# emma-mens/adam-compression

Hardware: AMD Instinct MI355X
Metric: grad elements/s per DGC step (HBM GB/s % of peak), 0.1% ratio, 1-8 GPUs (higher is better)
Workload: dtype f32

## Files before the change

adam-compression_amd/csrc/dgc_common.hpp:

```cpp
#pragma once

#include <hip/hip_runtime.h>
#include <hip/hip_fp16.h>

#include <cstdint>
#include <cstdio>
#include <string>

#include "dgc_hip.h"

namespace dgc {

void set_error(const char* fmt, ...);

#define DGC_FAIL(code, ...)            \
    do {                               \
        ::dgc::set_error(__VA_ARGS__); \
        return (code);                 \
    } while (0)

#define DGC_HIP(call)                                                                  \
    do {                                                                               \
        hipError_t _e = (call);                                                        \
        if (_e != hipSuccess)                                                          \
// ... 170 lines not shown

__host__ __device__ __forceinline__ float bf16_to_f32(uint16_t b) {
    union { uint32_t u; float f; } c{(uint32_t)b << 16};
    return c.f;
}
__host__ __device__ __forceinline__ uint16_t f32_to_bf16(float x) {
    union { float f; uint32_t u; } c{x};
    if ((c.u & 0x7FFFFFFFu) > 0x7F800000u) return (uint16_t)0x7FC0u;
    return (uint16_t)((c.u + 0x7FFFu + ((c.u >> 16) & 1u)) >> 16);
}
__device__ __forceinline__ float f16_to_f32(uint16_t h) { return (float)__builtin_bit_cast(_Float16, h); }
__device__ __forceinline__ uint16_t f32_to_f16(float x) {
    asm volatile("" : "+v"(x));
    return __builtin_bit_cast(uint16_t, (_Float16)x);
}
template <int DT>
__device__ __forceinline__ float h16_to_f32(uint16_t v) { return DT == DGC_BF16 ? bf16_to_f32(v) : f16_to_f32(v); }
template <int DT>
__device__ __forceinline__ uint16_t f32_to_h16(float x) { return DT == DGC_BF16 ? f32_to_bf16(x) : f32_to_f16(x); }
template <int DT>
__device__ __forceinline__ float round16(float x) { return h16_to_f32<DT>(f32_to_h16<DT>(x)); }
__device__ __forceinline__ float thr_mul(float t, float f, int td) {
    const float p = __fmul_rn(t, f);
    return td == DGC_BF16 ? round16<DGC_BF16>(p) : td == DGC_F16 ? round16<DGC_F16>(p) : p;
}

__device__ __forceinline__ void store_value(void* out, int64_t pos, float x, int vdtype) {
    if (vdtype == DGC_BF16)
        reinterpret_cast<uint16_t*>(out)[pos] = f32_to_bf16(x);
    else if (vdtype == DGC_F16)
        reinterpret_cast<__half*>(out)[pos] = __float2half_rn(x);
    else
        reinterpret_cast<float*>(out)[pos] = x;
}

__device__ __forceinline__ void store_index(void* out, int64_t pos, int64_t idx, int idtype) {
    if (idtype == DGC_I32)
        reinterpret_cast<int32_t*>(out)[pos] = (int32_t)idx;
    else
        reinterpret_cast<int64_t*>(out)[pos] = idx;
}

__device__ __forceinline__ uint64_t block_exclusive_scan(uint64_t v, uint64_t* lds16, uint64_t* total) {
    const int lane = threadIdx.x & 63, wid = threadIdx.x >> 6;
    const uint64_t incl = wave_incl_scan64(v);
    if (lane == 63) lds16[wid] = incl;
    __syncthreads();
    uint64_t wbase = 0, tot = 0;
    for (int w = 0; w < (int)(blockDim.x >> 6); ++w) {
        const uint64_t s = lds16[w];
        if (w < wid) wbase += s;
        tot += s;
    }
    __syncthreads();
    *total = tot;
    return wbase + incl - v;
}

}

namespace dgc {
typedef float f4v __attribute__((ext_vector_type(4)));

__device__ __forceinline__ float4 ld_nt(const float4* p) {
    const f4v x = __builtin_nontemporal_load(reinterpret_cast<const f4v*>(p));
    return make_float4(x[0], x[1], x[2], x[3]);
}

__device__ __forceinline__ void st_nt(float4* p, const float4& v) {
    const f4v x = {v.x, v.y, v.z, v.w};
    __builtin_nontemporal_store(x, reinterpret_cast<f4v*>(p));
}

constexpr int64_t kWriteThroughMax = 48LL << 20;
inline bool write_through(int64_t elements) { return elements <= kWriteThroughMax; }

__device__ __forceinline__ void st_stream(float4* p, const float4& v, bool wt) {
    if (wt) {
        const f4v x = {v.x, v.y, v.z, v.w};
        asm volatile("global_store_dwordx4 %0, %1, off sc1\n\ts_nop 1" : : "v"(p), "v"(x) : "memory");
    } else {
        st_nt(p, v);
    }
}
}

namespace dgc {
struct SampleSpec {
    float* out;
    int64_t start;
    int64_t stride;
    int64_t count;
    double inv_stride;
    float inv_stride_f;
};

__device__ __forceinline__ void divmod_u32(uint32_t t, uint32_t s, float inv, uint32_t& q, uint32_t& r) {
    if (s < (1u << 23)) {
        q = (uint32_t)__fmul_rn((float)t, inv);
        int32_t rr = (int32_t)(t - q * s);
        if (rr < 0) {
            q -= 1;
            rr += (int32_t)s;
        } else if (rr >= (int32_t)s) {
            q += 1;
            rr -= (int32_t)s;
        }
        r = (uint32_t)rr;
    } else {
        q = t / s;
        r = t - q * s;
    }
}

__device__ __forceinline__ void floor_divmod_fast(int64_t d, int64_t s, double inv, int64_t& q, int64_t& r) {
    q = (int64_t)floor((double)d * inv);
    r = d - q * s;
    while (r < 0) {
        r += s;
        q -= 1;
    }
    while (r >= s) {
        r -= s;
        q += 1;
    }
}

template <bool NEST, bool ACC>
__device__ __forceinline__ float comp1(float g, float& m, float& v, float mom) {
    if (NEST) {
        m = __fmul_rn(__fadd_rn(m, g), mom);
        if (ACC) {
            v = __fadd_rn(__fadd_rn(v, m), g);
            return v;
        }
        return __fadd_rn(m, g);
    }
    m = __fadd_rn(__fmul_rn(m, mom), g);
    if (ACC) {
        v = __fadd_rn(v, m);
        return v;
    }
    return m;
}

struct ClipArg {
    const float* tab;
    float value;
};

__host__ __device__ inline bool clip_kind_ok(int kind) { return kind >= DGC_CLIP_NONE && kind <= DGC_CLIP_CLAMP; }

template <int CLIP>
__device__ __forceinline__ float clip_coef(const ClipArg& ca, int t) {
    if (CLIP == DGC_CLIP_NONE) return 0.f;
    return ca.tab ? ca.tab[t] : ca.value;
}

template <int CLIP>
__device__ __forceinline__ float clip1(float g, float c) {
    if (CLIP == DGC_CLIP_SCALE) return c < 1.f ? __fmul_rn(g, c) : g;
    if (CLIP == DGC_CLIP_CLAMP) return c != c ? c : (g != g ? g : fminf(fmaxf(g, -c), c));
    return g;
}

template <int CLIP>
// ... 93 lines not shown
```

adam-compression_amd/csrc/select.hip:

```cpp
#include <algorithm>
#include <cstdlib>
#include <cstring>
#include <cmath>
#include <vector>

#include "select_types.hpp"
#include "select_layout.hpp"
#include "select_tiles.hpp"
#include "select_k1.hpp"
#include "select_state.hpp"
#include "select_thresholds.hpp"
#include "select_count.hpp"
#include "select_emit.hpp"
#include "select_heap.hpp"
#include "select_set.hpp"
#include "select_nth.hpp"

namespace dgc {

int64_t payload_layout(int64_t capacity, int vd, int id, int64_t* voff, int64_t* ioff);

__global__ void k_spec_reset(float* spec, int32_t T) {
    for (int i = threadIdx.x; i < kSpecWords * T; i += blockDim.x) spec[i] = __builtin_huge_valf();
}
// ... 316 lines not shown
    OneTable ot{};
    one_layout(*p, 1, 1, false, L, ot);
    SelWS w;
    DGC_TRY(carve_checked(ws, ws_bytes, L, "dgc_select", w));
    w.spec = nullptr;
    w.thr = const_cast<float*>(thr0);
    hipLaunchKernelGGL(k_put_one, dim3(1), dim3(64), 0, s, w, ot);
    DGC_LAUNCHED();
    return select_core(vec, mmt, cfg_of(*p), L, values, indices, count_out, info, w, 0, sync_mode, 1.f,
                       p->status_sink, p->order_out, s);
}

static size_t kth_ws_bytes(int64_t n) { return n <= kSmallN ? 256 : align_up(sizeof(RSState), 256); }

int kth_largest(const float* x, int64_t n, int64_t k, float* out, void* ws, size_t ws_bytes, hipStream_t s) {
    if (!x || !out || n < 1 || k < 1 || k > n)
        DGC_FAIL(DGC_ERR_INVALID, "dgc_kth_largest: need 1 <= k <= n (k=%lld n=%lld)", (long long)k,
                 (long long)n);
    if (n <= kSmallN) {
        hipLaunchKernelGGL(k_rs_small, dim3(1), dim3(kScanThreads), 0, s, x, n, (uint64_t)k, out);
        DGC_LAUNCHED();
        return DGC_OK;
    }
    if (!ws || ws_bytes < sizeof(RSState) || (reinterpret_cast<uintptr_t>(ws) & 255))
        DGC_FAIL(DGC_ERR_WORKSPACE, "dgc_kth_largest: workspace needs %zu bytes", sizeof(RSState));
    RSState* st = reinterpret_cast<RSState*>(ws);
    hipLaunchKernelGGL(k_rs_init, dim3(1), dim3(kBlock), 0, s, st, (uint64_t)k);
    DGC_LAUNCHED();
    return radix_select_passes(DenseKeys{x, n, st, out}, grid_for(n, kBlock * 16, 512), s);
}

static int thresholds(const SelWS& w, const Layout& L, const float* vec, hipStream_t s, int64_t ks1 = 0) {
    if (L.nsmall + L.nwins) {
        hipLaunchKernelGGL(k_rs_small_multi, dim3((unsigned)(L.nsmall + L.nwins)), dim3(kScanThreads), 0, s, w, vec,
                           ks1, L.nsmall);
        DGC_LAUNCHED();
    }
    if (L.grid[BT_SAMP] > 0) {
        if (L.nplain) {
            hipLaunchKernelGGL(k_rs_reset_samples, dim3((unsigned)L.T), dim3(kBlock), 0, s, w, ks1);
            DGC_LAUNCHED();
        }
        const int grid = (int)L.grid[BT_SAMP];
        hipLaunchKernelGGL(k_rs_passes<SampleKeys>, dim3((unsigned)std::min(grid, 1024)), dim3(kBlock), 0, s,
                           SampleKeys{w, vec}, grid, (int)L.T);
        DGC_LAUNCHED();
    }
    return DGC_OK;
}

int compensate(const float* grad, float* mmt, float* vec, float* out, int64_t n, float momentum,
               bool nesterov, bool accumulate, float* samples, int64_t s_start, int64_t s_stride,
               int64_t s_count, hipStream_t st);
int compensate_clip(const float* grad, float* mmt, float* vec, float* out, int64_t n, float momentum,
                    bool nesterov, bool accumulate, float* samples, int64_t s_start, int64_t s_stride,
                    int64_t s_count, int32_t clip_kind, ClipArg ca, hipStream_t st);
int sample_strided_launch(const float* vec, int64_t start, int64_t stride, int64_t count, float* out,
                          hipStream_t s);

static int compress_check(const dgc_select_params* p, void* values, void* indices, int64_t s_start,
                          int64_t s_stride, int64_t top_k_samples, bool need_outputs) {
    if (need_outputs) DGC_TRY(validate_select(p, values, indices));
    else if (!p) DGC_FAIL(DGC_ERR_INVALID, "dgc_compress: null params");
    else if (p->resample) DGC_TRY(check_replay_width(p->numel, p->num_selects, "dgc_compress"));
    const bool sampled = p->numel != p->num_samples;
    if (sampled && (s_stride < 2 || s_start < 0 || s_start >= s_stride))
        DGC_FAIL(DGC_ERR_INVALID, "dgc_compress: sample_start must be in [0, stride)");
    const int64_t cnt = sampled ? ceil_div(p->numel - s_start, s_stride) : p->numel;
    if (need_outputs && (top_k_samples < 1 || top_k_samples > cnt))
        DGC_FAIL(DGC_ERR_INVALID, "dgc_compress: top_k_samples %lld outside [1, %lld]", (long long)top_k_samples,
                 (long long)cnt);
    return DGC_OK;
}

static int one_ws(const dgc_select_params* p, int64_t s_start, int64_t s_stride, int64_t ks, float* spec,
                  void* ws, size_t ws_bytes, Layout& L, SelWS& w, OneTable& ot) {
    one_layout(*p, s_stride, ks, true, L, ot);
    ot.start = p->numel != p->num_samples ? s_start : 0;
    DGC_TRY(carve_checked(ws, ws_bytes, L, "dgc_compress", w));
    w.spec = spec;
    return DGC_OK;
}

template <bool NEST, bool ONE, typename... Args>
static void launch_k1_clip(int32_t clip_kind, dim3 gd, hipStream_t s, Args... args) {
    if (clip_kind == DGC_CLIP_SCALE)
        hipLaunchKernelGGL((k_compensate_list<NEST, ONE, DGC_CLIP_SCALE>), gd, dim3(kBlock), 0, s, args...);
    else if (clip_kind == DGC_CLIP_CLAMP)
        hipLaunchKernelGGL((k_compensate_list<NEST, ONE, DGC_CLIP_CLAMP>), gd, dim3(kBlock), 0, s, args...);
    else
        hipLaunchKernelGGL((k_compensate_list<NEST, ONE, DGC_CLIP_NONE>), gd, dim3(kBlock), 0, s, args...);
}

template <bool ONE, typename... Args>
static void launch_k1(bool nesterov, int32_t clip_kind, dim3 gd, hipStream_t s, Args... args) {
    if (nesterov) launch_k1_clip<true, ONE>(clip_kind, gd, s, args...);
    else launch_k1_clip<false, ONE>(clip_kind, gd, s, args...);
}

static int k1_clip_check(int32_t kind, const float* clip, const char* who) {
    if (!clip_kind_ok(kind)) DGC_FAIL(DGC_ERR_INVALID, "%s: clip kind %d", who, (int)kind);
    if (kind == DGC_CLIP_SCALE && !clip) DGC_FAIL(DGC_ERR_INVALID, "%s: DGC_CLIP_SCALE needs the coefficient table", who);
    return DGC_OK;
}

int compress_begin(const float* grad, float* mmt, float* vec, float momentum, bool nesterov, int64_t s_start,
                   int64_t s_stride, const dgc_select_params* p, float* spec, void* ws, size_t ws_bytes,
                   hipStream_t s, int32_t clip_kind = DGC_CLIP_NONE, ClipArg ca = ClipArg{nullptr, 0.f}) {
    DGC_TRY(compress_check(p, nullptr, nullptr, s_start, s_stride, 1, false));
    DGC_TRY(k1_clip_check(clip_kind, ca.tab, "dgc_compress"));
    if (!grad || !mmt || !vec) DGC_FAIL(DGC_ERR_INVALID, "dgc_compress: null grad/mmt/vec");
    Layout L;
    SelWS w;
    OneTable ot{};
    DGC_TRY(one_ws(p, s_start, s_stride, 1, spec, ws, ws_bytes, L, w, ot));
    const int64_t n = p->numel;
    const bool sampled = n != p->num_samples;
    const int64_t cnt = sampled ? ceil_div(n - s_start, s_stride) : 0;
    const bool list_path = aligned16(grad) && aligned16(mmt) && aligned16(vec) &&
                           (!sampled || (s_stride >= 4 && s_stride < (1LL << 30)));
    if (!list_path) {
        hipLaunchKernelGGL(k_put_one, dim3(1), dim3(64), 0, s, w, ot);
        DGC_LAUNCHED();
        DGC_TRY(mask_flush(vec, mmt, L, w, s));
        DGC_TRY(compensate_clip(grad, mmt, vec, nullptr, n, momentum, nesterov, true, sampled ? w.samples : nullptr,
                                s_start, s_stride, cnt, clip_kind, ca, s));
        hipLaunchKernelGGL(k_no_lists, dim3(1), dim3(64), 0, s, w);
        DGC_LAUNCHED();
        return DGC_OK;
    }
    if (L.grid[BT_K1] > 0x7FFFFFFFLL) DGC_FAIL(DGC_ERR_INVALID, "dgc_compress: n too large");
    if (L.grid[BT_K1] > 0) {
        StartChunk one{};
        one.count = 1;
        one.start[0] = ot.start;
        launch_k1<true>(nesterov, clip_kind, dim3((unsigned)L.grid[BT_K1]), s, grad, mmt, vec, momentum, w, one,
                        (int)write_through(n), ot, ca);
        DGC_LAUNCHED();
    } else {
        hipLaunchKernelGGL(k_put_one, dim3(1), dim3(64), 0, s, w, ot);
        DGC_LAUNCHED();
    }
    if (n & 3) {
        const int64_t done = (n / 4) * 4;
        DGC_TRY(compensate_clip(grad + done, mmt + done, vec + done, nullptr, n - done, momentum, nesterov, true,
                                nullptr, 0, 1, 0, clip_kind, ca, s));
        if (sampled) {
            const int64_t q_first = done >= s_start ? ceil_div(done - s_start, s_stride) : 0;
            const int64_t c = cnt - q_first;
            if (c > 0)
                DGC_TRY(sample_strided_launch(vec, s_start + q_first * s_stride, s_stride, c, w.samples + q_first, s));
        }
    }
    return DGC_OK;
}

int compress_finish(float* vec, float* mmt, int64_t s_start, int64_t s_stride, int64_t top_k_samples,
                    const dgc_select_params* p, float* spec, float margin, void* values, void* indices,
                    int64_t* count_out, dgc_select_info* info, void* ws, size_t ws_bytes, int sync_mode,
                    hipStream_t s) {
    DGC_TRY(compress_check(p, values, indices, s_start, s_stride, top_k_samples, true));
    if (!vec || (p->masking && !mmt)) DGC_FAIL(DGC_ERR_INVALID, "dgc_compress: null vec/mmt");
    Layout L;
    SelWS w;
    OneTable ot{};
    DGC_TRY(one_ws(p, s_start, s_stride, top_k_samples, spec, ws, ws_bytes, L, w, ot));
    DGC_TRY(thresholds(w, L, vec, s, top_k_samples));
    dgc_select_params q = *p;
    q.update_memory = p->update_memory == 2 ? 2 : 1;
    return select_core(vec, mmt, cfg_of(q), L, values, indices, count_out, info, w, 1, sync_mode, margin,
                       p->status_sink, p->order_out, s);
}

static int batch_layout(const dgc_batch_desc* b, HostTables& h) {
    if (!b || b->count < 1 || !b->numel || !b->offset || !b->num_selects || !b->num_samples || !b->top_k_samples ||
        !b->sample_stride)
        DGC_FAIL(DGC_ERR_INVALID, "dgc_batch: null or empty tensor table");
    std::vector<TensorIn> in(b->count);
    int64_t prev_end = 0;
    for (int32_t t = 0; t < b->count; ++t) {
        TensorIn& x = in[t];
        x.n = b->numel[t];
        x.off = b->offset[t];
        x.k = b->num_selects[t];
        x.S = b->num_samples[t];
        x.ks = b->top_k_samples[t];
        x.stride = b->sample_stride[t];
        x.upper_count = (int64_t)std::floor((double)x.k * b->upper_bound);
        x.lower_count = (int64_t)std::ceil(b->lower_bound * (double)x.k);
        x.samples = true;
        if (x.n < 1 || x.k < 1 || x.k > x.n || x.S < 1 || x.S > x.n || x.ks < 1 || x.ks > x.S)
            DGC_FAIL(DGC_ERR_INVALID, "dgc_batch: tensor %d: bad numel/num_selects/num_samples/top_k_samples", t);
        if (b->resample) {
            char who[48];
            std::snprintf(who, sizeof(who), "dgc_batch: tensor %d", t);
            DGC_TRY(check_replay_width(x.n, x.k, who));
        }
        if (x.n != x.S && (x.stride < 4 || x.stride >= (1LL << 30)))
            DGC_FAIL(DGC_ERR_INVALID, "dgc_batch: tensor %d: sample stride %lld outside [4, 2^30)", t,
                     (long long)x.stride);
        if (x.off % kSeg || x.off < prev_end)
            DGC_FAIL(DGC_ERR_INVALID,
                     "dgc_batch: tensor %d: offset %lld must be a multiple of %d, ascending, non-overlapping", t,
                     (long long)x.off, kSeg);
        prev_end = x.off + (int64_t)align_up((size_t)x.n, 4);
        if (prev_end > b->flat_numel) DGC_FAIL(DGC_ERR_INVALID, "dgc_batch: tensor %d past flat_numel", t);
    }
    if (b->int32_indices && b->flat_numel > 2147483647LL)
        DGC_FAIL(DGC_ERR_OVERFLOW, "dgc_batch: int32 indices cannot address %lld elements", (long long)b->flat_numel);
    if (b->dtype != DGC_F32 && b->dtype != DGC_BF16 && b->dtype != DGC_F16)
        DGC_FAIL(DGC_ERR_DTYPE, "dgc_batch: dtype must be DGC_F32, DGC_BF16 or DGC_F16");
    h.build(in.data(), b->count, true);
    return DGC_OK;
}

static SelCfg cfg_of_batch(const dgc_batch_desc* b) {
    const bool half = b->dtype == DGC_BF16 || b->dtype == DGC_F16;
    return SelCfg{(float)b->upper_bound, (float)b->lower_bound, b->max_iters, b->resample, b->momentum_masking,
                  b->fp16_values ? DGC_F16 : (half ? b->dtype : DGC_F32), b->int32_indices ? DGC_I32 : DGC_I64,
                  half ? 0 : (b->deferred_masking ? 2 : 1), half ? b->dtype : DGC_F32,
// ... 15 lines not shown
}

int batch_init(const dgc_batch_desc* b, void* ws, size_t ws_bytes, hipStream_t s) {
    HostTables h;
    SelWS w;
    DGC_TRY(batch_ws(b, ws, ws_bytes, "dgc_batch_init", h, w));
    const Layout& L = h.L;
    DGC_HIP(hipMemsetAsync(w.st, 0, sizeof(SelState) * L.T, s));
    DGC_HIP(hipMemsetAsync(w.setg, 0, sizeof(SetG) * L.T, s));
    DGC_HIP(hipMemsetAsync(w.chain, 0, kChainWords * sizeof(uint32_t), s));
    DGC_HIP(hipMemsetAsync(w.samples, 0, sizeof(float) * L.nsamp, s));
    DGC_HIP(hipMemcpyAsync(w.td, h.td.data(), sizeof(TDesc) * L.T, hipMemcpyHostToDevice, s));
    for (int which = 0; which < BT_COUNT; ++which)
        DGC_HIP(hipMemcpyAsync(w.bt[which], h.bt[which].data(), sizeof(int32_t) * (L.T + 1), hipMemcpyHostToDevice, s));
    if (L.nsmall + L.nwins)
        DGC_HIP(hipMemcpyAsync(w.small, h.small.data(), sizeof(int32_t) * (L.nsmall + L.nwins),
                               hipMemcpyHostToDevice, s));
    hipLaunchKernelGGL(k_spec_reset, dim3(1), dim3(256), 0, s, w.spec, L.T);
    DGC_LAUNCHED();
    DGC_HIP(hipStreamSynchronize(s));
    return DGC_OK;
}

static int check_starts(const HostTables& h, const int64_t* starts, const char* who) {
    for (int32_t t = 0; t < h.L.T; ++t)
        if (h.td[t].samp_off >= 0 && (starts[t] < 0 || starts[t] >= h.td[t].stride))
            DGC_FAIL(DGC_ERR_INVALID, "%s: tensor %d: sample start outside [0, stride)", who, t);
    return DGC_OK;
}

static StartChunk start_chunk(const HostTables& h, const int64_t* starts, const float* const* grads, int32_t first) {
    StartChunk c{};
    c.first = first;
    c.count = std::min<int32_t>(64, h.L.T - first);
    c.ptrs = grads ? 1 : 0;
    for (int i = 0; i < c.count; ++i) {
        c.start[i] = h.td[first + i].samp_off >= 0 ? starts[first + i] : 0;
        c.grad[i] = grads ? grads[first + i] : nullptr;
    }
    return c;
}

static int put_starts(const HostTables& h, const int64_t* starts, const float* const* grads, const SelWS& w,
                      hipStream_t s) {
    for (int32_t t0 = 0; t0 < h.L.T; t0 += 64) {
        hipLaunchKernelGGL(k_put_starts, dim3(1), dim3(64), 0, s, w, start_chunk(h, starts, grads, t0));
        DGC_LAUNCHED();
    }
    return DGC_OK;
}

static int batch_select_core(const dgc_batch_desc* b, const SelCfg& cfg, const HostTables& h, float* vec, float* mmt,
                             void* payload, dgc_select_info* info, const SelWS& w, int sync_mode, hipStream_t s) {
    int64_t cap = 0;
    for (const TDesc& d : h.td) cap += d.k;
    int64_t voff = 0, ioff = 0;
    payload_layout(cap, cfg.vdtype, cfg.idtype, &voff, &ioff);
    char* pl = static_cast<char*>(payload);
    return select_core(vec, mmt, cfg, h.L, pl + voff, pl + ioff, reinterpret_cast<int64_t*>(pl), info, w, 1,
                       sync_mode, b->spec_margin, b->status_sink, reinterpret_cast<int64_t*>(pl) + 1, s);
}

int batch_compress_begin(const dgc_batch_desc* b, const float* grad, const float* const* grads, float* mmt,
                         float* vec, const int64_t* starts, void* ws, size_t ws_bytes, hipStream_t s,
                         int32_t clip_kind = DGC_CLIP_NONE, ClipArg ca = ClipArg{nullptr, 0.f}) {
    HostTables h;
    SelWS w;
    DGC_TRY(k1_clip_check(clip_kind, ca.tab, "dgc_batch_compress"));
    DGC_TRY(batch_ws(b, ws, ws_bytes, "dgc_batch_compress", h, w));
    const Layout& L = h.L;
    if ((!grad && !grads) || !mmt || !vec || !starts) DGC_FAIL(DGC_ERR_INVALID, "dgc_batch_compress: null pointer");
    if ((grad && !aligned16(grad)) || !aligned16(mmt) || !aligned16(vec))
        DGC_FAIL(DGC_ERR_INVALID, "dgc_batch_compress: flat buffers must be 16-B aligned");
    if (grads)
        for (int32_t t = 0; t < L.T; ++t)
            if (!grads[t] || !aligned16(grads[t]))
                DGC_FAIL(DGC_ERR_INVALID, "dgc_batch_compress: gradient %d is null or not 16-B aligned", t);
    DGC_TRY(check_starts(h, starts, "dgc_batch_compress"));
    StartChunk arg{};
    arg.ptrs = grads ? 1 : 0;
    if (L.T <= 64) arg = start_chunk(h, starts, grads, 0);
    else DGC_TRY(put_starts(h, starts, grads, w, s));
    if (L.grid[BT_K1] > 0x7FFFFFFFLL) DGC_FAIL(DGC_ERR_INVALID, "dgc_batch_compress: too many segments");
    launch_k1<false>(b->nesterov != 0, clip_kind, dim3((unsigned)L.grid[BT_K1]), s, grad, mmt, vec, b->momentum, w, arg,
                     (int)write_through(L.nseg * kSeg), OneTable{}, ca);
    DGC_LAUNCHED();
    return DGC_OK;
}

int batch_compress_finish(const dgc_batch_desc* b, float* mmt, float* vec, void* payload, dgc_select_info* info,
                          void* ws, size_t ws_bytes, int sync_mode, hipStream_t s) {
    HostTables h;
    SelWS w;
    DGC_TRY(batch_ws(b, ws, ws_bytes, "dgc_batch_compress", h, w));
    if (!mmt || !vec || !payload) DGC_FAIL(DGC_ERR_INVALID, "dgc_batch_compress: null pointer");
    DGC_TRY(thresholds(w, h.L, vec, s));
    return batch_select_core(b, cfg_of_batch(b), h, vec, mmt, payload, info, w, sync_mode, s);
}

__global__ void __launch_bounds__(kBlock) k_batch_sample(SelWS w, const float* __restrict__ x_flat) {
    const int t = blockIdx.y;
    const TDesc d = w.td[t];
    if (d.samp_off < 0) return;
    const int64_t start = w.starts[t], cnt = w.scnt[t];
    const float* x = x_flat + d.off + start;
    float* out = w.samples + d.samp_off;
    for (int64_t q = (int64_t)blockIdx.x * kBlock + threadIdx.x; q < cnt; q += (int64_t)gridDim.x * kBlock)
        out[q] = fabsf(x[q * d.stride]);
}

int batch_select(const dgc_batch_desc* b, float* vec32, float* mmt32, const int64_t* starts, void* payload,
                 dgc_select_info* info, void* ws, size_t ws_bytes, int sync_mode, hipStream_t s) {
    HostTables h;
    SelWS w;
    DGC_TRY(batch_ws(b, ws, ws_bytes, "dgc_batch_select", h, w));
    const Layout& L = h.L;
    if (!vec32 || !starts || !payload) DGC_FAIL(DGC_ERR_INVALID, "dgc_batch_select: null pointer");
    const SelCfg cfg = cfg_of_batch(b);
    if (cfg.update_memory && cfg.masking && !mmt32) DGC_FAIL(DGC_ERR_INVALID, "dgc_batch_select: masking needs mmt");
    DGC_TRY(check_starts(h, starts, "dgc_batch_select"));
    DGC_TRY(put_starts(h, starts, nullptr, w, s));
    int64_t smax = 0;
    for (const TDesc& d : h.td) smax = std::max(smax, d.samp_off >= 0 ? d.S + 1 : 0);
    if (smax > 0) {
        hipLaunchKernelGGL(k_batch_sample, dim3((unsigned)std::min<int64_t>(ceil_div(smax, (int64_t)kBlock), 1024),
                                                (unsigned)L.T), dim3(kBlock), 0, s, w, vec32);
        DGC_LAUNCHED();
    }
    hipLaunchKernelGGL(k_no_lists, dim3(1), dim3(256), 0, s, w);
    DGC_LAUNCHED();
    DGC_TRY(thresholds(w, L, vec32, s));
    return batch_select_core(b, cfg, h, vec32, mmt32, payload, info, w, sync_mode, s);
}

int batch_compress(const dgc_batch_desc* b, const float* grad, float* mmt, float* vec, const int64_t* starts,
                   void* payload, dgc_select_info* info, void* ws, size_t ws_bytes, int sync_mode, hipStream_t s) {
    if (!payload) DGC_FAIL(DGC_ERR_INVALID, "dgc_batch_compress: null pointer");
    DGC_TRY(batch_compress_begin(b, grad, nullptr, mmt, vec, starts, ws, ws_bytes, s));
    return batch_compress_finish(b, mmt, vec, payload, info, ws, ws_bytes, sync_mode, s);
}

int compress_flush(float* vec, float* mmt, int64_t s_stride, const dgc_select_params* p, void* ws, size_t ws_bytes,
                   hipStream_t s) {
    if (!p || !vec) DGC_FAIL(DGC_ERR_INVALID, "dgc_compress_flush: null params/vec");
    Layout L;
    SelWS w;
    OneTable ot{};
    DGC_TRY(one_ws(p, 0, s_stride, 1, nullptr, ws, ws_bytes, L, w, ot));
    return mask_flush(vec, mmt, L, w, s);
}

int batch_flush(const dgc_batch_desc* b, float* mmt, float* vec, void* ws, size_t ws_bytes, hipStream_t s) {
    HostTables h;
    SelWS w;
    DGC_TRY(batch_ws(b, ws, ws_bytes, "dgc_batch_flush", h, w, vec && mmt));
    return mask_flush(vec, mmt, h.L, w, s);
}

}

extern "C" size_t dgc_kth_largest_workspace(int64_t n) { return dgc::kth_ws_bytes(n); }

extern "C" int dgc_kth_largest(const float* x, int64_t n, int64_t k, float* thr_out, void* ws,
                               size_t ws_bytes, void* stream) {
    return dgc::kth_largest(x, n, k, thr_out, ws, ws_bytes, static_cast<hipStream_t>(stream));
}

// ... 154 lines not shown
```

adam-compression_amd/csrc/select_k1.hpp:

```cpp
#pragma once
#include "select_tiles.hpp"

namespace dgc {
template <bool NEST, bool ONE, int CLIP>
__global__ void __launch_bounds__(kBlock)
k_compensate_list(const float* __restrict__ g_flat, float* __restrict__ mmt_flat, float* __restrict__ vec_flat,
                  float mom, SelWS w, StartChunk sc, int wt, OneTable ot, ClipArg ca) {
    const int t = ONE ? 0 : task(w, BT_K1, blockIdx.x);
    const TDesc d = ONE ? ot.d : w.td[t];
    const int lane = threadIdx.x & 63, wave = threadIdx.x >> 6;
    const int64_t b0 = ONE ? 0 : w.bt[BT_K1][t];
    const int64_t ls = ((int64_t)blockIdx.x - b0) * kSegPerBlock4 + wave;
    if (ONE && blockIdx.x == 0 && threadIdx.x == 0) {
        w.td[0] = ot.d;
        for (int which = 0; which < BT_COUNT; ++which) {
            w.bt[which][0] = ot.bt[which][0];
            w.bt[which][1] = ot.bt[which][1];
        }
        w.small[0] = 0;
    }
    const bool arg_start = t < sc.count;
    const float* gsrc = !sc.ptrs ? g_flat + d.off : (arg_start ? sc.grad[t] : w.gptr[t]);
    const float4* g = reinterpret_cast<const float4*>(gsrc);
    float4* mmt = reinterpret_cast<float4*>(mmt_flat + d.off);
    float4* vec = reinterpret_cast<float4*>(vec_flat + d.off);
    const int64_t n4 = d.nv4, n = d.n;
    const float tl = w.spec ? w.spec[kSpecWords * t] : __builtin_huge_valf();
    SelState* st = w.st + t;
    if (blockIdx.x == b0 && threadIdx.x == 0) st->t_list = tl;
    const bool sample = d.samp_off >= 0;
    const int64_t start = !sample ? 0 : (arg_start ? sc.start[t] : w.starts[t]);
    const int64_t scount = !sample ? 0 : (arg_start ? ceil_div(d.n - start, d.stride) : w.scnt[t]);
    if (arg_start && blockIdx.x == b0 && threadIdx.x == 0) {
        w.starts[t] = sc.start[t];
        w.scnt[t] = sample ? scount : d.n;
    }
    float* sout = sample ? w.samples + d.samp_off : nullptr;
    float* win = w.samples + d.win_off;
    const float tw = w.spec ? w.spec[kSpecWords * t + 2] : __builtin_huge_valf();
    const uint32_t win_key = abs_key(tw < __builtin_huge_valf() ? tw : tl);
    const bool windowed = sample && d.win_cap > 0;
    uint32_t* win_cnt = &st->win_cnt[st->epoch & 1];
    uint32_t* whist = reinterpret_cast<uint32_t*>(w.samples + d.whist_off);
    if (windowed && blockIdx.x == b0 && threadIdx.x == 0) st->win_key = win_key;
    int64_t q0 = 0, r0 = 0;
    if (sample) floor_divmod_fast(ls * kSeg - start, d.stride, d.inv_stride, q0, r0);
    float4 gv[kSegTiles], mv[kSegTiles], vv[kSegTiles];
    const float cf = clip_coef<CLIP>(ca, t);
#pragma unroll
    for (int u = 0; u < kSegTiles; ++u) {
        const int64_t v = ls * (kSeg / 4) + u * 64 + lane;
        if (v < n4) {
            gv[u] = clip4<CLIP>(sc.ptrs && 4 * v + 3 >= n ? ld_tail4(gsrc, 4 * v, n) : ld_nt(g + v), cf);
            mv[u] = ld_nt(mmt + v);
            vv[u] = ld_nt(vec + v);
        }
    }
    uint32_t c = 0, mk = 0;
    const int64_t seg = d.seg0 + ls;
    uint16_t* lo = w.lst_off;
    float* lv = w.lst_val;
    if (st->def_mode && ls < d.nseg) apply_deferred_mask(*st, w, d, ls, lane, vv, mv);
#pragma unroll
    for (int u = 0; u < kSegTiles; ++u) {
        const int64_t v = ls * (kSeg / 4) + u * 64 + lane;
        const bool ok = v < n4;
        float x[4] = {0.f, 0.f, 0.f, 0.f};
        uint32_t valid = 0;
        bool hit = false;
        float hv = 0.f;
        if (ok) {
            x[0] = comp1<NEST, true>(gv[u].x, mv[u].x, vv[u].x, mom);
            x[1] = comp1<NEST, true>(gv[u].y, mv[u].y, vv[u].y, mom);
            x[2] = comp1<NEST, true>(gv[u].z, mv[u].z, vv[u].z, mom);
            x[3] = comp1<NEST, true>(gv[u].w, mv[u].w, vv[u].w, mom);
            st_stream(mmt + v, mv[u], wt);
            st_stream(vec + v, vv[u], wt);
            const int64_t e = 4 * v;
            valid = e + 3 < n ? 0xFu : (e + 2 < n ? 7u : (e + 1 < n ? 3u : (e < n ? 1u : 0u)));
            if (sample) {
                const uint32_t tt = (uint32_t)r0 + 4u * (uint32_t)(u * 64 + lane);
                const uint32_t s32 = (uint32_t)d.stride;
                uint32_t q1, r;
                divmod_u32(tt, s32, d.inv_stride_f, q1, r);
                const uint32_t j = r == 0 ? 0u : s32 - r;
                if (j < 4 && ((valid >> j) & 1u)) {
                    const int64_t qi = q0 + q1 + (r == 0 ? 0 : 1);
                    if (qi >= 0 && qi < scount) {
                        hv = fabsf(x[j]);
                        sout[qi] = hv;
                        hit = windowed && __float_as_uint(hv) >= win_key;
                    }
                }
            }
        }
        const uint64_t hb = __ballot(hit);
        if (hb) {
            const int leader = __ffsll((unsigned long long)hb) - 1;
            uint32_t base = 0;
            if (lane == leader) base = atomicAdd(win_cnt, (uint32_t)__popcll(hb));
            base = __shfl(base, leader);
            const uint32_t pos = base + (uint32_t)__popcll(hb & ((1ull << lane) - 1));
            if (hit && pos < (uint64_t)d.win_cap) win[pos] = hv;
            if (hit) atomicAdd(&whist[win_bin(__float_as_uint(hv), win_key)], 1u);
        }
        list_append(ge_mask(x, valid, tl), x, u * 256, c, lo, lv, seg);
        mk = max(mk, tile_max_key(x, valid));
    }
    const bool spilled = c > (uint32_t)kCap;
    mk = wave_max(mk);
    if (lane == 0 && ls < d.nseg) {
        const bool tail = d.tail && ls == d.nseg - 1;
        w.seg_lcnt[seg] = tail ? lcnt_pack(kCap + 1, 0xFFFFu) : lcnt_pack(c, lmax_code(mk));
    }
    const uint64_t any = __ballot(spilled);
    __shared__ uint32_t nsp;
    if (threadIdx.x == 0) nsp = 0;
    __syncthreads();
    if (lane == 0 && any) atomicAdd(&nsp, 1u);
    __syncthreads();
    if (threadIdx.x == 0 && nsp) atomicAdd(&st->spill[st->epoch & 1][blockIdx.x % kSpillShards], nsp);
}

__global__ void k_no_lists(SelWS w) {
    for (int t = threadIdx.x; t < w.T; t += blockDim.x) w.st[t].t_list = __builtin_huge_valf();
}
}
```

adam-compression_amd/csrc/select_tiles.hpp:

```cpp
#pragma once
#include "select_layout.hpp"

namespace dgc {
__device__ __forceinline__ float4 ld_tail4(const float* __restrict__ g, int64_t e0, int64_t n) {
    if (e0 + 3 < n) return ld_nt(reinterpret_cast<const float4*>(g + e0));
    return make_float4(g[e0], e0 + 1 < n ? g[e0 + 1] : 0.f, e0 + 2 < n ? g[e0 + 2] : 0.f, 0.f);
}

__device__ __forceinline__ uint32_t lmax_code(uint32_t max_key) { return (max_key >> 16) + 1; }
__device__ __forceinline__ uint32_t lcnt_pack(uint32_t count, uint32_t code) { return count | (code << 16); }
__device__ __forceinline__ uint32_t lcnt_count(uint32_t v) { return v & 0xFFFFu; }
__device__ __forceinline__ uint32_t tile_max_key(const float (&x)[4], uint32_t valid) {
    uint32_t m = 0;
#pragma unroll
    for (int j = 0; j < 4; ++j)
        if ((valid >> j) & 1u) m = max(m, abs_key(x[j]));
    return m;
}

template <bool ALIGNED>
__device__ __forceinline__ void load_tile(const float* __restrict__ v, int64_t n, int64_t e0, float (&x)[4],
                                          uint32_t& valid) {
    if (ALIGNED && e0 + 3 < n) {
        const float4 q = ld_nt(reinterpret_cast<const float4*>(v + e0));
        x[0] = q.x;
        x[1] = q.y;
        x[2] = q.z;
        x[3] = q.w;
        valid = 0xFu;
    } else {
        valid = 0;
#pragma unroll
        for (int j = 0; j < 4; ++j) {
            const bool ok = e0 + j < n;
            x[j] = ok ? v[e0 + j] : 0.f;
            valid |= (uint32_t)ok << j;
        }
    }
}

__device__ __forceinline__ uint32_t ge_mask(const float (&x)[4], uint32_t valid, float t) {
    uint32_t p = 0;
#pragma unroll
    for (int j = 0; j < 4; ++j) p |= (uint32_t)(fabsf(x[j]) >= t) << j;
    return p & valid;
}

__device__ __forceinline__ void list_append(uint32_t p, const float (&x)[4], int tile_off, uint32_t& c,
                                            uint16_t* lo, float* lv, int64_t seg) {
    if (__ballot(p != 0)) {
        uint32_t lb, tot;
        wave_prefix4(p, lb, tot);
        uint32_t r = c + lb;
        const int lane = threadIdx.x & 63;
#pragma unroll
        for (int j = 0; j < 4; ++j) {
            if (p & (1u << j)) {
                if (r < (uint32_t)kCap) {
                    lo[lslot(seg, r)] = (uint16_t)(tile_off + 4 * lane + j);
                    lv[lslot(seg, r)] = x[j];
                }
                ++r;
            }
        }
        c += tot;
    }
}

__device__ __forceinline__ void load_segment(const float* __restrict__ v, int64_t n, int64_t ls,
                                             float (&x)[kSegTiles][4], uint32_t (&valid)[kSegTiles]) {
    const int lane = threadIdx.x & 63;
    if (aligned16(v)) {
#pragma unroll
        for (int u = 0; u < kSegTiles; ++u) load_tile<true>(v, n, ls * kSeg + u * 256 + 4 * lane, x[u], valid[u]);
    } else {
#pragma unroll
        for (int u = 0; u < kSegTiles; ++u) load_tile<false>(v, n, ls * kSeg + u * 256 + 4 * lane, x[u], valid[u]);
    }
}

__device__ uint32_t wave_count_segment(const float* __restrict__ v, int64_t n, int64_t ls, float t) {
    float x[kSegTiles][4];
    uint32_t valid[kSegTiles];
    load_segment(v, n, ls, x, valid);
    uint32_t c = 0;
#pragma unroll
    for (int u = 0; u < kSegTiles; ++u) c += __popc(ge_mask(x[u], valid[u], t));
    return wave_sum(c);
}

__device__ __forceinline__ int task(const SelWS& w, int which, int b) { return task_of_block(w.bt[which], w.T, b); }

__device__ __forceinline__ void apply_deferred_mask(const SelState& st, const SelWS& w, const TDesc& d,
                                                    int64_t ls, int lane, float4 (&vv)[kSegTiles],
                                                    float4 (&mv)[kSegTiles]) {
    const float dt = st.def_t;
    const long long dlim = st.def_limit;
    const bool mm = st.def_mask_mmt != 0;
    long long rank = w.grp_off[d.grp0 + ls / kGroupSegs] + w.seg_off[d.seg0 + ls];
#pragma unroll
    for (int u = 0; u < kSegTiles; ++u) {
        if (rank >= dlim) break;
        const int64_t v = ls * (kSeg / 4) + u * 64 + lane;
        const float xo[4] = {vv[u].x, vv[u].y, vv[u].z, vv[u].w};
        const uint32_t pm = ge_mask(xo, v < d.nv4 ? 0xFu : 0u, dt);
        uint32_t lb, tot;
        wave_prefix4(pm, lb, tot);
        long long r = rank + lb;
        float* vf = reinterpret_cast<float*>(&vv[u]);
        float* mf = reinterpret_cast<float*>(&mv[u]);
#pragma unroll
        for (int j = 0; j < 4; ++j)
            if (pm & (1u << j)) {
                if (r < dlim) {
                    vf[j] = 0.f;
                    if (mm) mf[j] = 0.f;
                }
                ++r;
            }
        rank += tot;
    }
}

__global__ void __launch_bounds__(kBlock) k_mask_flush(float* __restrict__ vec_flat, float* __restrict__ mmt_flat,
                                                       SelWS w) {
    const int t = task(w, BT_K1, blockIdx.x);
    const SelState* st = w.st + t;
    if (!st->def_mode) return;
    const TDesc d = w.td[t];
    const int lane = threadIdx.x & 63, wave = threadIdx.x >> 6;
    const int64_t ls = ((int64_t)blockIdx.x - w.bt[BT_K1][t]) * kSegPerBlock4 + wave;
    if (ls >= d.nseg) return;
    float* vec = vec_flat + d.off;
    float* mmt = st->def_mask_mmt ? mmt_flat + d.off : nullptr;
    const float dt = st->def_t;
    const long long dlim = st->def_limit;
    long long rank = w.grp_off[d.grp0 + ls / kGroupSegs] + w.seg_off[d.seg0 + ls];
    if (rank >= dlim) return;
    float x[kSegTiles][4];
    uint32_t valid[kSegTiles];
    load_segment(vec, d.n, ls, x, valid);
#pragma unroll
    for (int u = 0; u < kSegTiles; ++u) {
        const uint32_t pm = ge_mask(x[u], valid[u], dt);
        uint32_t lb, tot;
        wave_prefix4(pm, lb, tot);
        long long r = rank + lb;
        const int64_t e0 = ls * kSeg + u * 256 + 4 * lane;
#pragma unroll
        for (int j = 0; j < 4; ++j)
            if (pm & (1u << j)) {
                if (r < dlim) {
                    vec[e0 + j] = 0.f;
                    if (mmt) mmt[e0 + j] = 0.f;
                }
                ++r;
            }
        rank += tot;
    }
}

__global__ void k_def_clear(SelWS w) {
    for (int t = threadIdx.x; t < w.T; t += blockDim.x) w.st[t].def_mode = 0;
}

static int mask_flush(float* vec, float* mmt, const Layout& L, const SelWS& w, hipStream_t s) {
    if (L.grid[BT_K1] > 0x7FFFFFFFLL) DGC_FAIL(DGC_ERR_INVALID, "dgc_compress: n too large");
    if (L.grid[BT_K1] > 0) {
        hipLaunchKernelGGL(k_mask_flush, dim3((unsigned)L.grid[BT_K1]), dim3(kBlock), 0, s, vec, mmt, w);
        DGC_LAUNCHED();
    }
    hipLaunchKernelGGL(k_def_clear, dim3(1), dim3(256), 0, s, w);
    DGC_LAUNCHED();
    return DGC_OK;
}
}
```

Baseline: 283.2 billion.

## Restructure K1 compensate kernel: hoist state loads, wave-level task lookup, drop block sync

The compensate-and-list kernel now finds its task with a wave-ballot scan, issues all per-task state, offset and spec loads up front, and loads momentum/vector before the gradient using address-space-qualified global pointers. The shared-memory spill reduction with two __syncthreads is replaced by a per-wave atomic. For large non-write-through tensors it requests 48KB of dynamic LDS to cap occupancy on the streaming pass. The aim is to cut load latency and barrier stalls in the memory-bound kernel. In exchange it adds more global atomics and lowers occupancy, which could hurt latency hiding.

```diff
diff --git a/adam-compression_amd/csrc/dgc_common.hpp b/adam-compression_amd/csrc/dgc_common.hpp
--- a/adam-compression_amd/csrc/dgc_common.hpp
+++ b/adam-compression_amd/csrc/dgc_common.hpp
@@ -276,6 +276,19 @@
     } else {
         st_nt(p, v);
     }
+}
+
+__device__ __forceinline__ float4 ld_nt(DGC_GLB const float4* p) {
+    const f4v x = __builtin_nontemporal_load(reinterpret_cast<DGC_GLB const f4v*>(p));
+    return make_float4(x[0], x[1], x[2], x[3]);
+}
+
+__device__ __forceinline__ void st_stream(DGC_GLB float4* p, const float4& v, bool wt) {
+    const f4v x = {v.x, v.y, v.z, v.w};
+    if (wt)
+        asm volatile("global_store_dwordx4 %0, %1, off sc1\n\ts_nop 1" : : "v"(p), "v"(x) : "memory");
+    else
+        __builtin_nontemporal_store(x, reinterpret_cast<DGC_GLB f4v*>(p));
 }
 }
 
diff --git a/adam-compression_amd/csrc/select.hip b/adam-compression_amd/csrc/select.hip
--- a/adam-compression_amd/csrc/select.hip
+++ b/adam-compression_amd/csrc/select.hip
@@ -422,20 +422,22 @@
     return DGC_OK;
 }
 
+constexpr unsigned kK1FlatLds = 48u << 10;
+
 template <bool NEST, bool ONE, typename... Args>
-static void launch_k1_clip(int32_t clip_kind, dim3 gd, hipStream_t s, Args... args) {
+static void launch_k1_clip(int32_t clip_kind, unsigned lds, dim3 gd, hipStream_t s, Args... args) {
     if (clip_kind == DGC_CLIP_SCALE)
-        hipLaunchKernelGGL((k_compensate_list<NEST, ONE, DGC_CLIP_SCALE>), gd, dim3(kBlock), 0, s, args...);
+        hipLaunchKernelGGL((k_compensate_list<NEST, ONE, DGC_CLIP_SCALE>), gd, dim3(kBlock), lds, s, args...);
     else if (clip_kind == DGC_CLIP_CLAMP)
-        hipLaunchKernelGGL((k_compensate_list<NEST, ONE, DGC_CLIP_CLAMP>), gd, dim3(kBlock), 0, s, args...);
+        hipLaunchKernelGGL((k_compensate_list<NEST, ONE, DGC_CLIP_CLAMP>), gd, dim3(kBlock), lds, s, args...);
     else
-        hipLaunchKernelGGL((k_compensate_list<NEST, ONE, DGC_CLIP_NONE>), gd, dim3(kBlock), 0, s, args...);
+        hipLaunchKernelGGL((k_compensate_list<NEST, ONE, DGC_CLIP_NONE>), gd, dim3(kBlock), lds, s, args...);
 }
 
 template <bool ONE, typename... Args>
-static void launch_k1(bool nesterov, int32_t clip_kind, dim3 gd, hipStream_t s, Args... args) {
-    if (nesterov) launch_k1_clip<true, ONE>(clip_kind, gd, s, args...);
-    else launch_k1_clip<false, ONE>(clip_kind, gd, s, args...);
+static void launch_k1(bool nesterov, int32_t clip_kind, unsigned lds, dim3 gd, hipStream_t s, Args... args) {
+    if (nesterov) launch_k1_clip<true, ONE>(clip_kind, lds, gd, s, args...);
+    else launch_k1_clip<false, ONE>(clip_kind, lds, gd, s, args...);
 }
 
 static int k1_clip_check(int32_t kind, const float* clip, const char* who) {
@@ -474,8 +476,9 @@
         StartChunk one{};
         one.count = 1;
         one.start[0] = ot.start;
-        launch_k1<true>(nesterov, clip_kind, dim3((unsigned)L.grid[BT_K1]), s, grad, mmt, vec, momentum, w, one,
-                        (int)write_through(n), ot, ca);
+        const bool wt = write_through(n);
+        launch_k1<true>(nesterov, clip_kind, wt ? 0u : kK1FlatLds, dim3((unsigned)L.grid[BT_K1]), s, grad, mmt, vec,
+                        momentum, w, one, (int)wt, ot, ca);
         DGC_LAUNCHED();
     } else {
         hipLaunchKernelGGL(k_put_one, dim3(1), dim3(64), 0, s, w, ot);
@@ -657,7 +660,7 @@
     if (L.T <= 64) arg = start_chunk(h, starts, grads, 0);
     else DGC_TRY(put_starts(h, starts, grads, w, s));
     if (L.grid[BT_K1] > 0x7FFFFFFFLL) DGC_FAIL(DGC_ERR_INVALID, "dgc_batch_compress: too many segments");
-    launch_k1<false>(b->nesterov != 0, clip_kind, dim3((unsigned)L.grid[BT_K1]), s, grad, mmt, vec, b->momentum, w, arg,
+    launch_k1<false>(b->nesterov != 0, clip_kind, 0u, dim3((unsigned)L.grid[BT_K1]), s, grad, mmt, vec, b->momentum, w, arg,
                      (int)write_through(L.nseg * kSeg), OneTable{}, ca);
     DGC_LAUNCHED();
     return DGC_OK;
diff --git a/adam-compression_amd/csrc/select_k1.hpp b/adam-compression_amd/csrc/select_k1.hpp
--- a/adam-compression_amd/csrc/select_k1.hpp
+++ b/adam-compression_amd/csrc/select_k1.hpp
@@ -2,16 +2,91 @@
 #include "select_tiles.hpp"
 
 namespace dgc {
+__device__ __forceinline__ int task_first(const int32_t* blk, int T, int b, int64_t& b0) {
+    b0 = 0;
+    if (T <= 1) return 0;
+    const int lane = threadIdx.x & 63;
+    int cnt = 0;
+    uint32_t first = 0;
+    for (int i0 = 0; i0 < T; i0 += 64) {
+        const int i = i0 + lane;
+        const int32_t v = i < T ? blk[i] : 0x7FFFFFFF;
+        const bool le = v <= b;
+        const uint64_t m = __ballot(le);
+        cnt += __popcll(m);
+        first = max(first, le ? (uint32_t)v : 0u);
+        if (m != ~0ull) break;
+    }
+    b0 = wave_max(first);
+    return __builtin_amdgcn_readfirstlane(cnt - 1);
+}
+
+static_assert(offsetof(SelState, t0) == 0 && offsetof(SelState, t_list) == 2 * sizeof(float),
+              "K1's stand-in for a null spec reads SelState words 0 and 2");
 template <bool NEST, bool ONE, int CLIP>
 __global__ void __launch_bounds__(kBlock)
 k_compensate_list(const float* __restrict__ g_flat, float* __restrict__ mmt_flat, float* __restrict__ vec_flat,
                   float mom, SelWS w, StartChunk sc, int wt, OneTable ot, ClipArg ca) {
-    const int t = ONE ? 0 : task(w, BT_K1, blockIdx.x);
+    int64_t b0 = 0;
+    const int t = ONE ? 0 : task_first(w.bt[BT_K1], w.T, blockIdx.x, b0);
     const TDesc d = ONE ? ot.d : w.td[t];
-    const int lane = threadIdx.x & 63, wave = threadIdx.x >> 6;
-    const int64_t b0 = ONE ? 0 : w.bt[BT_K1][t];
+    const int lane = threadIdx.x & 63, wave = wave_id();
     const int64_t ls = ((int64_t)blockIdx.x - b0) * kSegPerBlock4 + wave;
-    if (ONE && blockIdx.x == 0 && threadIdx.x == 0) {
+    const bool live = ls < d.nseg;
+    const bool first = blockIdx.x == b0 && threadIdx.x == 0;
+    const bool arg_start = ONE || t < sc.count;
+    const bool ptrs = !ONE && sc.ptrs;
+    const bool sample = d.samp_off >= 0;
+
+    DGC_GLB SelState* st = glb(w.st + t);
+    DGC_GLB const float* spec = w.spec ? glb(w.spec + kSpecWords * t) : &st->t0;
+    const float spec0 = spec[0], spec2 = spec[2];
+    const int32_t epoch = st->epoch, def_mode = st->def_mode, def_mask_mmt = st->def_mask_mmt;
+    const float def_t = st->def_t;
+    const long long def_limit = st->def_limit;
+    const int64_t lsd = live ? ls : 0;
+    DGC_GLB const long long* grp_off = glb(w.grp_off) + (d.grp0 + lsd / kGroupSegs);
+    DGC_GLB const uint32_t* seg_off = glb(w.seg_off) + (d.seg0 + lsd);
+    long long def_rank = 0;
+    if (ONE) def_rank = *grp_off + (long long)*seg_off;
+    float cf_tab = 0.f;
+    if (CLIP != DGC_CLIP_NONE) cf_tab = *(ca.tab ? glb(ca.tab + t) : (DGC_GLB const float*)&st->t0);
+    int64_t start_ws = 0, scnt_ws = 0;
+    const float* gptr_ws = nullptr;
+    if (!arg_start) {
+        start_ws = glb(w.starts)[t];
+        scnt_ws = glb(w.scnt)[t];
+        if (ptrs) gptr_ws = glb(w.gptr)[t];
+    }
+
+    const int64_t n = d.n;
+    const int64_t seg4 = ls * (kSeg / 4);
+    const int left = (int)min(d.nv4 - seg4, (int64_t)(kSeg / 4));
+    const int gleft = ptrs ? (int)min((n >> 2) - seg4, (int64_t)(kSeg / 4)) : left;
+    DGC_GLB float4* mmt = glb(reinterpret_cast<float4*>(mmt_flat + d.off) + seg4);
+    DGC_GLB float4* vec = glb(reinterpret_cast<float4*>(vec_flat + d.off) + seg4);
+    const float* gsrc = !ptrs ? g_flat + d.off : (arg_start ? sc.grad[ONE ? 0 : t] : gptr_ws);
+    DGC_GLB const float4* g = glb(reinterpret_cast<const float4*>(gsrc) + seg4);
+    float4 gv[kSegTiles], mv[kSegTiles], vv[kSegTiles];
+#pragma unroll
+    for (int u = 0; u < kSegTiles; ++u) {
+        if (u * 64 + lane < left) {
+            mv[u] = ld_nt(mmt + u * 64 + lane);
+            vv[u] = ld_nt(vec + u * 64 + lane);
+        }
+    }
+#pragma unroll
+    for (int u = 0; u < kSegTiles; ++u)
+        if (u * 64 + lane < gleft) gv[u] = ld_nt(g + u * 64 + lane);
+    if (ptrs && gleft < left && gleft >= 0) {
+#pragma unroll
+        for (int u = 0; u < kSegTiles; ++u)
+            if (u * 64 + lane == gleft) gv[u] = ld_tail4(glb(gsrc), n);
+    }
+
+    if (!ONE) def_rank = *grp_off + (long long)*seg_off;
+
+    if (ONE && first) {
         w.td[0] = ot.d;
         for (int which = 0; which < BT_COUNT; ++which) {
             w.bt[which][0] = ot.bt[which][0];
@@ -19,64 +94,46 @@
         }
         w.small[0] = 0;
     }
-    const bool arg_start = t < sc.count;
-    const float* gsrc = !sc.ptrs ? g_flat + d.off : (arg_start ? sc.grad[t] : w.gptr[t]);
-    const float4* g = reinterpret_cast<const float4*>(gsrc);
-    float4* mmt = reinterpret_cast<float4*>(mmt_flat + d.off);
-    float4* vec = reinterpret_cast<float4*>(vec_flat + d.off);
-    const int64_t n4 = d.nv4, n = d.n;
-    const float tl = w.spec ? w.spec[kSpecWords * t] : __builtin_huge_valf();
-    SelState* st = w.st + t;
-    if (blockIdx.x == b0 && threadIdx.x == 0) st->t_list = tl;
-    const bool sample = d.samp_off >= 0;
-    const int64_t start = !sample ? 0 : (arg_start ? sc.start[t] : w.starts[t]);
-    const int64_t scount = !sample ? 0 : (arg_start ? ceil_div(d.n - start, d.stride) : w.scnt[t]);
-    if (arg_start && blockIdx.x == b0 && threadIdx.x == 0) {
-        w.starts[t] = sc.start[t];
+    const float tl = w.spec ? spec0 : __builtin_huge_valf();
+    const float cf = ca.tab ? cf_tab : ca.value;
+    if (first) st->t_list = tl;
+    const int64_t start = !sample ? 0 : (arg_start ? sc.start[ONE ? 0 : t] : start_ws);
+    const int64_t scount = !sample ? 0 : (arg_start ? ceil_div(d.n - start, d.stride) : scnt_ws);
+    if (arg_start && first) {
+        w.starts[t] = start;
         w.scnt[t] = sample ? scount : d.n;
     }
     float* sout = sample ? w.samples + d.samp_off : nullptr;
     float* win = w.samples + d.win_off;
-    const float tw = w.spec ? w.spec[kSpecWords * t + 2] : __builtin_huge_valf();
+    const float tw = w.spec ? spec2 : __builtin_huge_valf();
     const uint32_t win_key = abs_key(tw < __builtin_huge_valf() ? tw : tl);
     const bool windowed = sample && d.win_cap > 0;
-    uint32_t* win_cnt = &st->win_cnt[st->epoch & 1];
+    uint32_t* win_cnt = &w.st[t].win_cnt[epoch & 1];
     uint32_t* whist = reinterpret_cast<uint32_t*>(w.samples + d.whist_off);
-    if (windowed && blockIdx.x == b0 && threadIdx.x == 0) st->win_key = win_key;
+    if (windowed && first) st->win_key = win_key;
     int64_t q0 = 0, r0 = 0;
     if (sample) floor_divmod_fast(ls * kSeg - start, d.stride, d.inv_stride, q0, r0);
-    float4 gv[kSegTiles], mv[kSegTiles], vv[kSegTiles];
-    const float cf = clip_coef<CLIP>(ca, t);
-#pragma unroll
-    for (int u = 0; u < kSegTiles; ++u) {
-        const int64_t v = ls * (kSeg / 4) + u * 64 + lane;
-        if (v < n4) {
-            gv[u] = clip4<CLIP>(sc.ptrs && 4 * v + 3 >= n ? ld_tail4(gsrc, 4 * v, n) : ld_nt(g + v), cf);
-            mv[u] = ld_nt(mmt + v);
-            vv[u] = ld_nt(vec + v);
-        }
-    }
     uint32_t c = 0, mk = 0;
     const int64_t seg = d.seg0 + ls;
     uint16_t* lo = w.lst_off;
     float* lv = w.lst_val;
-    if (st->def_mode && ls < d.nseg) apply_deferred_mask(*st, w, d, ls, lane, vv, mv);
+    if (def_mode && live) apply_deferred_mask(def_t, def_limit, def_mask_mmt != 0, def_rank, d, ls, lane, vv, mv);
 #pragma unroll
     for (int u = 0; u < kSegTiles; ++u) {
-        const int64_t v = ls * (kSeg / 4) + u * 64 + lane;
-        const bool ok = v < n4;
+        const bool ok = u * 64 + lane < left;
         float x[4] = {0.f, 0.f, 0.f, 0.f};
         uint32_t valid = 0;
         bool hit = false;
         float hv = 0.f;
         if (ok) {
-            x[0] = comp1<NEST, true>(gv[u].x, mv[u].x, vv[u].x, mom);
-            x[1] = comp1<NEST, true>(gv[u].y, mv[u].y, vv[u].y, mom);
-            x[2] = comp1<NEST, true>(gv[u].z, mv[u].z, vv[u].z, mom);
-            x[3] = comp1<NEST, true>(gv[u].w, mv[u].w, vv[u].w, mom);
-            st_stream(mmt + v, mv[u], wt);
-            st_stream(vec + v, vv[u], wt);
-            const int64_t e = 4 * v;
+            const float4 gq = clip4<CLIP>(gv[u], cf);
+            x[0] = comp1<NEST, true>(gq.x, mv[u].x, vv[u].x, mom);
+            x[1] = comp1<NEST, true>(gq.y, mv[u].y, vv[u].y, mom);
+            x[2] = comp1<NEST, true>(gq.z, mv[u].z, vv[u].z, mom);
+            x[3] = comp1<NEST, true>(gq.w, mv[u].w, vv[u].w, mom);
+            st_stream(mmt + u * 64 + lane, mv[u], wt);
+            st_stream(vec + u * 64 + lane, vv[u], wt);
+            const int64_t e = 4 * (seg4 + u * 64 + lane);
             valid = e + 3 < n ? 0xFu : (e + 2 < n ? 7u : (e + 1 < n ? 3u : (e < n ? 1u : 0u)));
             if (sample) {
                 const uint32_t tt = (uint32_t)r0 + 4u * (uint32_t)(u * 64 + lane);
@@ -107,19 +164,12 @@
         list_append(ge_mask(x, valid, tl), x, u * 256, c, lo, lv, seg);
         mk = max(mk, tile_max_key(x, valid));
     }
-    const bool spilled = c > (uint32_t)kCap;
     mk = wave_max(mk);
-    if (lane == 0 && ls < d.nseg) {
+    if (lane == 0 && live) {
         const bool tail = d.tail && ls == d.nseg - 1;
         w.seg_lcnt[seg] = tail ? lcnt_pack(kCap + 1, 0xFFFFu) : lcnt_pack(c, lmax_code(mk));
+        if (c > (uint32_t)kCap) atomicAdd(&w.st[t].spill[epoch & 1][blockIdx.x % kSpillShards], 1u);
     }
-    const uint64_t any = __ballot(spilled);
-    __shared__ uint32_t nsp;
-    if (threadIdx.x == 0) nsp = 0;
-    __syncthreads();
-    if (lane == 0 && any) atomicAdd(&nsp, 1u);
-    __syncthreads();
-    if (threadIdx.x == 0 && nsp) atomicAdd(&st->spill[st->epoch & 1][blockIdx.x % kSpillShards], nsp);
 }
 
 __global__ void k_no_lists(SelWS w) {
diff --git a/adam-compression_amd/csrc/select_tiles.hpp b/adam-compression_amd/csrc/select_tiles.hpp
--- a/adam-compression_amd/csrc/select_tiles.hpp
+++ b/adam-compression_amd/csrc/select_tiles.hpp
@@ -2,9 +2,10 @@
 #include "select_layout.hpp"
 
 namespace dgc {
-__device__ __forceinline__ float4 ld_tail4(const float* __restrict__ g, int64_t e0, int64_t n) {
-    if (e0 + 3 < n) return ld_nt(reinterpret_cast<const float4*>(g + e0));
-    return make_float4(g[e0], e0 + 1 < n ? g[e0 + 1] : 0.f, e0 + 2 < n ? g[e0 + 2] : 0.f, 0.f);
+__device__ __forceinline__ float4 ld_tail4(DGC_GLB const float* g, int64_t n) {
+    DGC_GLB const float* p = g + (n & ~(int64_t)3);
+    const int r = (int)(n & 3);
+    return make_float4(p[0], r > 1 ? p[1] : 0.f, r > 2 ? p[2] : 0.f, 0.f);
 }
 
 __device__ __forceinline__ uint32_t lmax_code(uint32_t max_key) { return (max_key >> 16) + 1; }
@@ -91,13 +92,9 @@
 
 __device__ __forceinline__ int task(const SelWS& w, int which, int b) { return task_of_block(w.bt[which], w.T, b); }
 
-__device__ __forceinline__ void apply_deferred_mask(const SelState& st, const SelWS& w, const TDesc& d,
-                                                    int64_t ls, int lane, float4 (&vv)[kSegTiles],
+__device__ __forceinline__ void apply_deferred_mask(float dt, long long dlim, bool mm, long long rank,
+                                                    const TDesc& d, int64_t ls, int lane, float4 (&vv)[kSegTiles],
                                                     float4 (&mv)[kSegTiles]) {
-    const float dt = st.def_t;
-    const long long dlim = st.def_limit;
-    const bool mm = st.def_mask_mmt != 0;
-    long long rank = w.grp_off[d.grp0 + ls / kGroupSegs] + w.seg_off[d.seg0 + ls];
 #pragma unroll
     for (int u = 0; u < kSegTiles; ++u) {
         if (rank >= dlim) break;
```

New measurement: 287.1 billion, median of 6. 1.01x the previous value.
